# nikihowe/myriad

Hardware: AMD Instinct MI355X
Metric: converged trajopt solves/sec (batched), CARTPOLE collocation N=100 (higher is better)
Workload: dtype f64; 1 GPU; CARTPOLE HS collocation N=100, batch=4096 random x0 (weak), converged = status 0 and max|c|<=1e-8; global_batch=4096, parallelism=instances sharded over 1 GPU(s), one process per GPU

## Files before the change

### myriad_amd/csrc/hs_solver_fused.h

```cpp
#pragma once
#include <hip/hip_runtime.h>
#include "hs_solver_wave.h"

namespace myriad {

struct ParkArgs {
  int mode;
  int k1;
  const int* perm;
  const int* count;
  double* state;
  long stride;
};
constexpr int MYR_STATUS_PARKED_ = 5;

struct NodeBoard {
  unsigned long long cmd;
  unsigned int done;
  unsigned int xcc;
  unsigned int att;
  unsigned int pad_[27];
};
struct CoopArgs {
  NodeBoard* boards;
  double* pub;
  long pub_stride;
  int maxh;
  int* abort;
};
constexpr unsigned int MYR_COOP_RUNNING = 0x80000000u;
constexpr int MYR_COOP_EXIT = 15;
constexpr unsigned int MYR_COOP_GEN_MASK = 0x7fffu;
__device__ inline void coop_release() { asm volatile("s_waitcnt vmcnt(0) lgkmcnt(0)" ::: "memory"); }
__device__ inline void coop_acquire() { asm volatile("buffer_inv sc1\n\ts_waitcnt vmcnt(0)" ::: "memory"); }
#ifdef MYR_COOP_DEBUG
#define COOP_DBG(bit, ...) do { if ((MYR_COOP_DEBUG) & (bit)) printf(__VA_ARGS__); } while (0)
#else
#define COOP_DBG(bit, ...)
#endif
#ifdef MYR_COOP_TRACE
__device__ int* g_coop_trace;
#define COOP_TR(slot, val) do { if (g_coop_trace) __hip_atomic_store(g_coop_trace + blockIdx.x * 16 + (slot), (int)(val), __ATOMIC_RELAXED, __HIP_MEMORY_SCOPE_SYSTEM); } while (0)
#else
#define COOP_TR(slot, val)
#endif
__device__ inline unsigned int coop_xcc_id() { return __builtin_amdgcn_s_getreg((31 << 11) | 20) & 15u; }
constexpr unsigned MYR_COOP_SPIN_MAX = 1u << 23;

#ifdef MYR_PHASE_TIMING
__device__ long long node_tph_[8];
__device__ long long bw_tph_[4];
#define MYR_BW_PH(i) { if (blockIdx.x == 0 && c.tid == 0) { const long long t1_ = clock64(); bw_tph_[i] += t1_ - bw_t0_; bw_t0_ = t1_; } }
#else
#define MYR_BW_PH(i)
#endif

template <class Sys, int W = 1, int SCHEME = 0>
struct HsFused {
  static constexpr int NT = 64 * W;
  static constexpr bool TRAP = SCHEME == 1;
  using W0 = HsWave<Sys, 0>;
  using S = HsSolver<Sys>;
  using D = HsSol<Sys>;
  static constexpr int NS = D::NS, NU = D::NU, NW = D::NW, NY = TRAP ? NS + 2 * NU : D::NY, NQ = TRAP ? NU : D::NQ, NC = D::NC, NY1 = NY + 1;
  static constexpr int QE = NQ - NU;
#ifndef MYR_FWD_SEQ_NW
#define MYR_FWD_SEQ_NW 7
#endif
#ifndef MYR_TL_FLOOR
#define MYR_TL_FLOOR 1e-10
#endif
  static constexpr bool TL = W > 1 && NU == 1 && NS <= 4;
  static constexpr int MLAM = TRAP ? 1 : 2;
  static constexpr bool MLP = NodeTraits<Sys>::mlp;
  static_assert(!(MLP && TRAP), "network dynamics are built for the Hermite-Simpson transcription");
  static constexpr int PT_F = 0, PT_A = PT_F + NS, PT_B = PT_A + NS * NS, PT_D2 = PT_B + NS * NU, PT_N = PT_D2 + NW * (NW + 1) / 2;
  static constexpr int HSYM = NW * (NW + 1) / 2;
  static constexpr int HR_H = 0, HR_G0 = HSYM, HR_G1 = HR_G0 + NW, HR_N = HR_G1 + NW;
  static constexpr int SG_GE = 0, SG_GM = NS * NY1, SG_N = (TRAP ? 1 : 2) * NS * NY1;
  static constexpr int KST = NQ * NW + NQ * NC, KSTR = KST;
  static constexpr int ZR = 32;
  static constexpr int PF = MYR_RICCATI_PF;
  static constexpr int PADH = PF * 2 * HR_N, PADS = PF * SG_N;
  __host__ __device__ static constexpr int symidx(int r, int c) { return r <= c ? r * NW - r * (r - 1) / 2 + (c - r) : c * NW - c * (c - 1) / 2 + (r - c); }
  __host__ __device__ static constexpr int npoints(int N) { return TRAP ? N + 1 : 2 * N + 1; }
  __host__ __device__ static inline double wq(int K, int j, double h) {
    if (TRAP) return (j == 0 || j == K - 1) ? 0.5 * h : h;
    return S::wsimp(K, j, h);
  }
  __host__ __device__ static inline double tq(int j, double h) { return TRAP ? h * j : 0.5 * h * j; }

  __host__ __device__ static long off_hr(int) { return ZR + PADH; }
  __host__ __device__ static long off_st(int N) { return off_hr(N) + (long)npoints(N) * HR_N + PADS; }
  __host__ __device__ static long off_kg(int N) { return off_st(N) + (long)N * SG_N; }
  __host__ __device__ static long off_lam(int N) { return off_kg(N) + (long)N * KST; }
  __host__ __device__ static long off_kg2(int N) { return off_lam(N) + (long)MLAM * N * NS; }
  __host__ __device__ static long off_pt(int N) { return off_kg2(N) + (W > 1 ? (long)N * KST : 0); }
  __host__ __device__ static long off_hb(int N) { return off_pt(N) + (MLP ? (long)PT_N * npoints(N) : 0); }
  __host__ __device__ static long off_mb(int N) { return off_hb(N) + (MLP ? (long)NodeMfma64::ntiles(npoints(N)) * NodeMfma64::HB_TILE : 0); }
  __host__ __device__ static long off_zlu(int N) { return off_mb(N) + (MLP ? (long)NodeMfma64::ntiles(npoints(N)) * NodeMfma64::MB_TILE : 0); }
  static constexpr bool FSEQ = (MYR_FWD_SEQ_NW > 0) && NW >= MYR_FWD_SEQ_NW && !MLP;
  static constexpr int FWS = NW * NW + NW;
  __host__ __device__ static long off_fw(int N) { return off_zlu(N) + (ZLU_GLOBAL ? 2L * npoints(N) * NW : 0); }
  __host__ __device__ static long scratch_doubles(int N) { return off_fw(N) + (FSEQ ? (long)N * FWS : 0); }
  static constexpr int NREC = NS + NS + NS * NS + NS * NU + NS;
  static constexpr int EXCH = NW * NW + NW * NC + NS * NC + NU * NC;
  static constexpr int NTOT = NW * NW + NW, NRED = 12;
  static constexpr int XCH = 2 * W * NREC + 2 * W * NTOT + 2 * W * 2 * NS + W * NRED + 8;
  static constexpr int NCH = W;
  static constexpr int NXB = TL ? NCH : (W > 1 ? 2 : 1);
  static constexpr int TL_TH1 = NCH * NC, TL_JN1 = (NCH - 1) * 4 * NW * NW;
  static constexpr int TL_TH = TL ? TL_TH1 + (NCH + 1) + 2 : 0, TL_JN = TL ? TL_JN1 : 0;
  __host__ __device__ static constexpr int lds_solver_doubles_z(int N, bool zlu_global) { return (zlu_global ? 2 : 4) * npoints(N) * NW + MLAM * N * NS + 6 * NW + XCH + NXB * EXCH + TL_TH + TL_JN + 8; }
  static constexpr bool ZLU_GLOBAL = (MLP && W == 2) ||
      (!MLP && (MYR_FWD_SEQ_NW > 0) && NW >= MYR_FWD_SEQ_NW && (long)lds_solver_doubles_z(100, false) * 8 > 40960L * W);
  __host__ __device__ static int lds_solver_doubles(int N) { return lds_solver_doubles_z(N, ZLU_GLOBAL); }
  __host__ __device__ static int lds_doubles(int N) { return lds_solver_doubles(N) + (MLP ? npoints(N) * NS + NodeTraits<Sys>::lds_doubles : 0); }
  __host__ __device__ static size_t lds_bytes(int N) { return (size_t)lds_doubles(N) * 8; }
  static constexpr int NSCAL = 48;
  __host__ __device__ static long park_doubles(int N) { return NSCAL + lds_solver_doubles(N) + (ZLU_GLOBAL ? 2L * npoints(N) * NW : 0); }

  struct Ctx {
    int N, K, n, lane, wave, tid;
    double h, h6, h8;
    double *z, *zL, *zU, *dz;
    double *hr, *st, *kg, *zr;
    double *fw;
    double *kgA, *kgB, *xA, *xB;
    double *sTh, *sJn;
    double *pt, *sF, *wl;
    double *hb, *mb;
    int nh, hidx;
    unsigned int gen;
    NodeBoard* board; int* coop_abort;
    double *pubx, *publam, *pubf;
    bool h_valid;
    const double *lb, *ub;
    bool uni;
    SysParams<Sys> pp;
    bool term_pinned[NS];
    double *sLam, *sB, *sStash, *sTot, *sTr, *sRed, *sMisc, *sP, *sPc, *sTnu, *sKu;
#ifdef MYR_PHASE_TIMING
    long long tph[16], t0;
#endif
#ifdef MYR_TRACE
    int traj;
#endif
  };
  __device__ static inline long zi(const Ctx& c, int j, int comp) { return S::zi(c.K, j, comp); }
  __device__ static inline void use_set(Ctx& c, double* kg, double* x) {
    c.kg = kg; c.sP = x; c.sPc = x + NW * NW; c.sTnu = c.sPc + NW * NC; c.sKu = c.sTnu + NS * NC;
  }
  __device__ static inline void wsync() {
    __syncthreads();
  }
  template <int NV>
  __device__ static inline void wg_combine(Ctx& c, double* v, const int (&op)[NV]) {
    static_assert(NV <= NRED, "partial-sum slots");
    if constexpr (W > 1) {
#pragma unroll
      for (int i = 0; i < NV; ++i) c.sRed[c.wave * NRED + i] = v[i];
      __syncthreads();
#pragma unroll
      for (int i = 0; i < NV; ++i) {
        double r = c.sRed[i];
#pragma unroll
// ... 723 lines not shown
      for (int r = 0; r < NW; ++r) {
        const bool zr = last && r < NS && c.term_pinned[r < NS ? r : 0];
#pragma unroll
        for (int q = r; q < NW; ++q) {
          const bool zq = last && q < NS && c.term_pinned[q < NS ? q : 0];
          hr[HR_H + symidx(r, q)] = (zr || zq) ? 0.0 : (Wh[r * NW + q] + ((r == q) ? sig[r] : 0.0));
        }
        hr[HR_G0 + r] = zr ? 0.0 : (TL ? fma(mu_fold, g1v[r], wj * P.gw[r]) : wj * P.gw[r]);
        hr[HR_G1 + r] = zr ? 0.0 : g1v[r];
      }
      }
    }
    double v[1] = {wv_max(st_)};
    const int op[1] = {1};
    wg_combine<1>(c, v, op);
    stat = v[0];
  }

  __device__ static int riccati_first_point(Ctx& c, const HsSolveOpts& o, double delta, int nreg) {
    using namespace detail;
    const int lane = c.lane;
    const double* hr = c.hr;
    double Puu[NU * NU], ku[NU * NC], pun[NU * NS];
#pragma unroll
    for (int a = 0; a < NU; ++a) {
#pragma unroll
      for (int b = 0; b < NU; ++b) Puu[a * NU + b] = c.sP[(NS + a) * NW + NS + b] + hr[HR_H + symidx(NS + a, NS + b)] + ((a == b) ? delta : 0.0);
#pragma unroll
      for (int cc = 0; cc < NC; ++cc)
        ku[a * NC + cc] = c.sPc[(NS + a) * NC + cc] + (cc == 0 ? hr[HR_G0 + NS + a] : (cc == 1 ? hr[HR_G1 + NS + a] : 0.0));
#pragma unroll
      for (int i = 0; i < NS; ++i) pun[a * NS + i] = ku[a * NC + 2 + i];
    }
    nreg += chol_reg<NU>(Puu, o.reg_floor);
    chol_solve<NU, NC>(Puu, ku);
    wave_sync<true>();
    if (lane == 0) {
#pragma unroll
      for (int i = 0; i < NS; ++i)
#pragma unroll
        for (int cc = 0; cc < NC; ++cc) {
          double s = 0.0;
#pragma unroll
          for (int a = 0; a < NU; ++a) s += pun[a * NS + i] * ku[a * NC + cc];
          c.sTnu[i * NC + cc] -= s;
        }
#pragma unroll
      for (int i = 0; i < NU * NC; ++i) c.sKu[i] = ku[i];
    }
    wave_sync<true>();
    return nreg;
  }

  template <bool CHUNK>
  __device__ static int riccati_tile(Ctx& c, const HsSolveOpts& o, double delta, bool abort_on_reg, int k_lo_, int k_hi_, bool last_, double* xo) {
    using namespace detail;
    const int k_lo = CHUNK ? __builtin_amdgcn_readfirstlane(k_lo_) : 0, k_hi = __builtin_amdgcn_readfirstlane(CHUNK ? k_hi_ : c.N);
    const bool last = CHUNK ? last_ : true;
    static_assert(!CHUNK || (NC == NS + 2 && NU == 1), "slot 7 takes the control's multiplier");
    const int lane = c.lane;
    const int g = lane >> 4, j = lane & 15;
    const int scol = tile_scol<NS>(j), ycol = tile_ycol<NS, true>(j, scol), rcc = tile_rcc<NC>(j);
    const bool rowx = g < NS;
    const double* he = c.hr + (long)(2 * (k_hi - 1) + 2) * HR_N;
    const double* hm = he - HR_N;
    const double* st = c.st + (long)(k_hi - 1) * SG_N;
    auto hsel = [&](const double* rec, int row, bool on) -> const double* {
      if (!on) return c.zr;
      if (scol >= 0) return rec + HR_H + (scol <= row ? scol * NW - scol * (scol - 1) / 2 + (row - scol) : row * NW - row * (row - 1) / 2 + (scol - row));
      if (rcc == 0) return rec + HR_G0 + row;
      if constexpr (!CHUNK) { if (rcc == 1) return rec + HR_G1 + row; }
      return c.zr;
    };
    auto gsel = [&](int off) -> const double* {
      if (!rowx) return c.zr;
      if (ycol >= 0) return st + off + g * NY1 + ycol;
      if (rcc == 0) return st + off + g * NY1 + NY;
      return c.zr;
    };
    const double* ptr[6] = {hsel(he, g, rowx), hsel(he, NS, g < 2), gsel(SG_GE), hsel(hm, g, rowx), hsel(hm, NS, g < 2), gsel(SG_GM)};
    long stp[6];
#pragma unroll
    for (int q = 0; q < 6; ++q) stp[q] = (ptr[q] == c.zr) ? 0 : ((q == 2 || q == 5) ? (long)SG_N : 2L * HR_N);
    const bool pinr = rowx && (!last || c.term_pinned[rowx ? g : 0]);
    const double rho0 = last ? o.rho_term - delta : o.rho_term;
    double X0 = (pinr && scol == g) ? rho0 : ((pinr && rcc == 2 + g) ? 1.0 : 0.0);
    double X1 = (!last && g < 2) ? (scol == NS ? rho0 : (rcc == 1 ? 1.0 : 0.0)) : 0.0;
    const double dv0 = (rowx && scol == g) ? delta : 0.0, dv1 = (g < 2 && scol == NS) ? delta : 0.0;
    const TileMask<CHUNK, true> m(g, j, rcc);
    const int k_off = (g == 0 && scol >= 0 && j != 5) ? scol : ((g == 0 && rcc >= 0) ? NQ * NW + rcc : -1);
    const int k_str = k_off < 0 ? 1 : ((scol >= 0) ? NW : NC);
    double* k_ptr = k_off >= 0 ? c.kg + (long)(k_hi - 1) * KSTR + k_off : c.zr + ZR - 2;
    const long k_step = k_off >= 0 ? KSTR : 0;
    double reg_floor = o.reg_floor;
    asm volatile("" : "+v"(reg_floor));
    int nreg = 0;
    const bool abort_u = uniform_if<(W > 1)>(abort_on_reg);
    double in[PF][6];
#pragma unroll
    for (int u = 0; u < PF; ++u) {
#pragma unroll
      for (int q = 0; q < 6; ++q) { in[u][q] = *ptr[q]; ptr[q] -= stp[q]; }
      __builtin_amdgcn_sched_barrier(0);
    }
    mfma_d4 D1c = {0.0, 0.0, 0.0, 0.0}, Rmc = {0.0, 0.0, 0.0, 0.0};
    mfma_d4 Qm;
    double QmU;
    auto mid_part = [&](double n0, double n1, double Gm, const mfma_d4& Cup) -> mfma_d4 {
      const mfma_d4 Rm = tile_prod1<8>(n0 + dv0, n1 + dv1, Gm, m.f_a1, m.f_keep, m.f_shm, Cup);
      Qm = tile_mfma(Gm, Rm[0], mfma_d4{0.0, 0.0, 0.0, 0.0});
      QmU = Rm[1];
      return Rm;
    };
    mid_part(in[0][3], in[0][4], in[0][5], mfma_d4{0.0, 0.0, 0.0, 0.0});
    mfma_d4 D3 = {X0, X1, 0.0, 0.0};
    auto stage = [&](const int u) {
      X0 = D3[0] + (in[u][0] + dv0); X1 = fma(D3[1], m.f_x1, in[u][1] + dv1);
      const double G = in[u][2];
      const double nn0 = in[(u + 1) % PF][3], nn1 = in[(u + 1) % PF][4], nGm = in[(u + 1) % PF][5];
      const mfma_d4 D1 = tile_prod1<4>(X0, X1, G, m.f_a1, m.f_keep, m.f_she, D1c);
      D1c = D1;
      mfma_d4 C2 = tile_c2_hs(D3, D1, Qm, m.f_t1, m.f_t23);
      C2[3] += QmU;
      const mfma_d4 D2 = tile_mfma(G, D1[0], C2);
      Rmc = mid_part(nn0, nn1, nGm, Rmc);
      const TileGain2 gn = tile_gain2<(W > 1)>(D2, reg_floor, nreg, TileNoStop());
      k_ptr[0] = gn.kk0; k_ptr[k_str] = gn.kk1;
      k_ptr -= k_step;
      D3 = tile_update2(D2, gn.kk0, gn.kk1, m.f_a3m, m.f_a3e, g);
#pragma unroll
      for (int q = 0; q < 6; ++q) { in[u][q] = *ptr[q]; ptr[q] -= stp[q]; }
    };
    auto group = [&]() {
#pragma unroll
      for (int u = 0; u < PF; ++u) stage(u);
    };
    int kb = k_hi - 1;
    if (kb - k_lo >= PF - 1) {
      group();
      for (kb -= PF; kb - k_lo >= PF - 1; kb -= PF) {
        if (uniform_if<true>(nreg > 0 && abort_u)) return nreg;
        group();
      }
    }
#pragma unroll
    for (int u = 0; u < PF - 1; ++u) {
      if (kb - u < k_lo) break;
      stage(u);
    }
    if (uniform_if<true>(nreg > 0 && abort_u)) return nreg;
    if constexpr (!CHUNK) {
      tile_store_first<false, NS, NC>(D3, g, j, scol, rcc, rowx, c.sP, c.sPc, c.sTnu, [] { wave_sync<true>(); });
      return riccati_first_point(c, o, delta, nreg);
    } else {
      double* xP = xo; double* xPc = xo + NW * NW; double* xT = xPc + NW * NC;
      tile_store_first<true, NS, NC>(D3, g, j, scol, rcc, rowx, xP, xPc, xT, [] { wave_sync<true>(); });
      return nreg;
    }
  }

  static constexpr bool GEN = !(NU == 1 && NS <= 4);
  static constexpr bool G_BIG = NW > 8 || NQ > 8;
  static constexpr int G_QT = G_BIG ? 1 : 0;
  static constexpr int G_QS = G_BIG ? 16 : 8;
  static constexpr int G_NB = (NW + 3) / 4, G_NQB = (NQ + 3) / 4, G_NYT = G_QT + 1;
  static constexpr int G_FREE_LO = G_QS - NW, G_FREE_HI = 16 * (G_QT + 1) - G_QS - NQ;
  static constexpr int G_REST = NC - G_FREE_LO - G_FREE_HI;
  static constexpr int G_CT = G_QT + 1 + (G_REST > 0 ? 1 : 0);
  static constexpr bool GEN_OK = NW <= 14 && NQ <= 16 && (G_BIG ? G_FREE_LO : G_FREE_LO + G_FREE_HI) >= 2 && G_FREE_HI >= 0 && G_REST <= 16;
  static constexpr bool SUPPORTED = !GEN || GEN_OK;
  __host__ __device__ static constexpr int g_rhs_slot(int cc) {
    return cc < G_FREE_LO ? NW + cc : (cc - G_FREE_LO < G_FREE_HI ? G_QS + NQ + (cc - G_FREE_LO) : 16 * (G_QT + 1) + (cc - G_FREE_LO - G_FREE_HI));
  }
  __host__ __device__ static constexpr int g_slot_cc(int slot) {
    int cc = -1;
    if (slot < NW) cc = -1;
    else if (slot < G_QS) cc = slot - NW;
    else if (slot < G_QS + NQ) cc = -1;
    else if (slot < 16 * (G_QT + 1)) cc = G_FREE_LO + (slot - G_QS - NQ);
    else cc = G_FREE_LO + G_FREE_HI + (slot - 16 * (G_QT + 1));
    return cc < NC ? cc : -1;
  }
  __host__ __device__ static constexpr bool g_map_ok() {
    for (int cc = 0; cc < NC; ++cc)
      if (g_slot_cc(g_rhs_slot(cc)) != cc || g_rhs_slot(cc) >= 16 * G_CT) return false;
    return g_rhs_slot(0) < 16 && g_rhs_slot(1) < 16;
  }
  __device__ static int riccati_mfma_gen(Ctx& c, const HsSolveOpts& o, double delta, bool abort_on_reg) {
    using namespace detail;
    static_assert(GEN_OK && g_map_ok(), "slot map: w in front of the q, '1' and mu in the first column tile");
    constexpr int NB = G_NB, NQB = G_NQB, CT = G_CT, QT = G_QT, NYT = G_NYT;
    constexpr int QL = G_QS & 15;
    constexpr int QR = QL / 4;
    constexpr int PFG = G_BIG ? 2 : PF;
    constexpr int NL1 = NB * (1 + NYT);
    constexpr int NL = (TRAP ? 1 : 2) * NL1;
    constexpr int L_HE = 0, L_GE = NB, L_HM = NL1, L_GM = NL1 + NB;
    constexpr long H_STEP = TRAP ? (long)HR_N : 2L * HR_N;
    const int lane = c.lane, N = c.N;
    const int g = lane >> 4, j = lane & 15;
    int wc[CT], qc[CT], rc[CT], yc[NYT];
#pragma unroll
    for (int C = 0; C < CT; ++C) {
      const int slot = 16 * C + j;
      wc[C] = slot < NW ? slot : -1;
      qc[C] = (slot >= G_QS && slot < G_QS + NQ) ? slot - G_QS : -1;
      rc[C] = g_slot_cc(slot);
    }
#pragma unroll
    for (int C = 0; C < NYT; ++C) yc[C] = wc[C] >= 0 ? wc[C] : (qc[C] >= 0 ? NW + qc[C] : -1);
// ... 193 lines not shown
            }
        }
#pragma unroll
        for (int C = 0; C < CT; ++C)
#pragma unroll
          for (int b = 0; b < NQB; ++b) {
            double v = 0.0;
#pragma unroll
            for (int e = 0; e < 4; ++e)
              if (4 * b + e < NQ) v = (g == e) ? kk[C][4 * b + e] : v;
            kp[C][b][0] = v;
            kp[C][b] -= kstep[C][b];
          }
      }
    }
#pragma unroll
    for (int C = 0; C < CT; ++C) {
#pragma unroll
      for (int r = 0; r < NB; ++r) {
        const int row = 4 * r + g;
        if (row < NW && wc[C] >= 0) c.sP[row * NW + wc[C]] = Q[0][C][r];
        if (row < NW && rc[C] >= 0) c.sPc[row * NC + rc[C]] = Q[0][C][r];
      }
#pragma unroll
      for (int R = 0; R < CT; ++R)
#pragma unroll
        for (int r = 0; r < 4; ++r) {
          const int cc = g_slot_cc(16 * R + 4 * r + g);
          if (cc >= 2 && rc[C] >= 0) c.sTnu[(cc - 2) * NC + rc[C]] = Q[R][C][r];
        }
    }
    wave_sync<true>();
    {
      constexpr int s1 = g_rhs_slot(0);
      static_assert(s1 < 16, "row '1' in the first tile");
#pragma unroll
      for (int C = 0; C < CT; ++C)
        if (g == (s1 & 3) && rc[C] >= 2) c.sTnu[(rc[C] - 2) * NC + 0] += Q[0][C][s1 >> 2];
    }
    wave_sync<true>();
    return riccati_first_point(c, o, delta, nreg);
  }
  struct SwArgs { nd_glb *hr, *st, *zr, *kg; nd_lds* xs; int N, lane, pinned, abort; double reg_floor, rho_term, delta; };
  __device__ __attribute__((noinline)) static int sweep_call(SwArgs a) {
    Ctx c;
    c.N = a.N; c.lane = a.lane; c.hr = (double*)a.hr; c.st = (double*)a.st; c.zr = (double*)a.zr;
    use_set(c, (double*)a.kg, (double*)a.xs);
#pragma unroll
    for (int q = 0; q < NS; ++q) c.term_pinned[q] = ((a.pinned >> q) & 1) != 0;
    HsSolveOpts o;
    o.reg_floor = a.reg_floor; o.rho_term = a.rho_term;
    if constexpr (GEN) return riccati_mfma_gen(c, o, a.delta, a.abort != 0);
    else if constexpr (TRAP) return riccati_tile_trap<false>(c, o, a.delta, a.abort != 0, 0, 0, true, nullptr);
    else return riccati_tile<false>(c, o, a.delta, a.abort != 0, 0, 0, true, nullptr);
  }
  __device__ static inline int sweep(Ctx& c, const HsSolveOpts& o, double delta, bool abort_on_reg) {
#if !defined(MYR_SWEEP_CALL_W) || MYR_SWEEP_CALL_W
    constexpr bool CALL = true;
#else
    constexpr bool CALL = W == 1;
#endif
    if constexpr (!CALL) {
      if constexpr (GEN) return riccati_mfma_gen(c, o, delta, abort_on_reg);
      else if constexpr (TRAP) return riccati_tile_trap<false>(c, o, delta, abort_on_reg, 0, 0, true, nullptr);
      else return riccati_tile<false>(c, o, delta, abort_on_reg, 0, 0, true, nullptr);
    } else {
      SwArgs a;
      a.hr = (nd_glb*)c.hr; a.st = (nd_glb*)c.st; a.zr = (nd_glb*)c.zr; a.kg = (nd_glb*)c.kg; a.xs = (nd_lds*)c.sP;
      a.N = c.N; a.lane = c.lane; a.abort = abort_on_reg ? 1 : 0;
      a.pinned = 0;
#pragma unroll
      for (int q = 0; q < NS; ++q) a.pinned |= c.term_pinned[q] ? (1 << q) : 0;
      a.reg_floor = o.reg_floor; a.rho_term = o.rho_term; a.delta = delta;
      return sweep_call(a);
    }
  }

  template <bool CHUNK>
  __device__ static int riccati_tile_trap(Ctx& c, const HsSolveOpts& o, double delta, bool abort_on_reg, int k_lo_, int k_hi_, bool last_, double* xo) {
    using namespace detail;
    static_assert(!TRAP || NQ == 1, "one control");
    const int k_lo = CHUNK ? __builtin_amdgcn_readfirstlane(k_lo_) : 0, k_hi = __builtin_amdgcn_readfirstlane(CHUNK ? k_hi_ : c.N);
    const bool last = CHUNK ? last_ : true;
    const int lane = c.lane;
    const int g = lane >> 4, j = lane & 15;
    const int scol = tile_scol<NS>(j);
    const int ycol = scol >= 0 ? scol : ((j == 8 || j == 9) ? NW : -1);
    const int rcc = tile_rcc<NC>(j);
    const bool rowx = g < NS;
    const double* he = c.hr + (long)k_hi * HR_N;
    const double* st = c.st + (long)(k_hi - 1) * SG_N;
    auto hsel = [&](int row, bool on) -> const double* {
      if (!on) return c.zr;
      if (scol >= 0) return he + HR_H + (scol <= row ? scol * NW - scol * (scol - 1) / 2 + (row - scol) : row * NW - row * (row - 1) / 2 + (scol - row));
      if (rcc == 0) return he + HR_G0 + row;
      if constexpr (!CHUNK) { if (rcc == 1) return he + HR_G1 + row; }
      return c.zr;
    };
    const double* ptr[3] = {hsel(g, rowx), hsel(NS, g < 2),
                            !rowx ? c.zr : (ycol >= 0 ? st + SG_GE + g * NY1 + ycol : (rcc == 0 ? st + SG_GE + g * NY1 + NY : c.zr))};
    long stp[3];
#pragma unroll
    for (int q = 0; q < 3; ++q) stp[q] = (ptr[q] == c.zr) ? 0 : (q == 2 ? (long)SG_N : (long)HR_N);
    const bool pinr = rowx && (!last || c.term_pinned[rowx ? g : 0]);
    const double rho0 = last ? o.rho_term - delta : o.rho_term;
    const double X0i = (pinr && scol == g) ? rho0 : ((pinr && rcc == 2 + g) ? 1.0 : 0.0);
// ... 693 lines not shown
    wsync();
#pragma unroll
    for (int q = 0; q < NS; ++q) c.term_pinned[q] = !(c.sB[2 * NW + q] < c.sB[3 * NW + q]);
    res.status = 1; res.iters = o.max_iter;
    for (int it = it0; it <= o.max_iter; ++it) {
      if (park_mode == 1 && it == park_k1) {
        const int nl = lds_solver_doubles(c.N);
        for (int i = c.tid; i < nl; i += NT) __builtin_nontemporal_store(c.z[i], &sv[NSCAL + i]);
        if constexpr (ZLU_GLOBAL) {
          for (int i = c.tid; i < 2 * c.n; i += NT) __builtin_nontemporal_store(c.zL[i], &sv[NSCAL + nl + i]);
        }
        if (c.tid == 0) {
          s.save(sv, hist, pending);
          sv[PK_UNI] = c.uni ? 1.0 : 0.0;
          sv[PK_RES] = res.cost; sv[PK_RES + 1] = res.feas; sv[PK_RES + 2] = res.stat; sv[PK_RES + 3] = res.compl_;
        }
        res.status = MYR_STATUS_PARKED_; res.iters = it;
        return;
      }
      if constexpr (MLP) { if (c.board) coop_refresh(c); }
      BOut p1;
      { NuT nu_; for (int q = 0; q < NS; ++q) nu_.v[q] = s.nuT[q]; p1 = backward_pass(c, pending, nu_); }
      pending.on = false;
      c.h_valid = false;
      wsync();
      MYR_PH(0)
      double stat_raw;
      const double mu_hess = s.mu;
      stat_raw = hessian_pass(c, s.mu);
      wsync();
      MYR_PH(4)
      const double c1 = p1.c1, cinf = p1.cinf, sum_mult = p1.sum_mult;
      double delta = s.first_delta(o);
      int nreg = 0;
      {
        const IpKkt k = s.kkt(o, sum_mult + p1.sm, MLAM * c.N * NS + p1.nm, p1.f, stat_raw, p1.cmax, cinf);
        res.cost = p1.f; res.feas = cinf; res.stat = k.stat; res.compl_ = k.comp;
        if (__builtin_amdgcn_readfirstlane((int)!k.finite)) { res.status = 2; res.iters = it; return; }
        if (__builtin_amdgcn_readfirstlane((int)k.converged)) { res.status = 0; res.iters = it; return; }
        if (it == o.max_iter) break;
        s.barrier_update(o, k, cinf, p1.cmin, p1.cmax);
      }
#if !defined(MYR_FUSED_SPEC) || MYR_FUSED_SPEC
      constexpr bool SPEC = W > 1;
#else
      constexpr bool SPEC = false;
#endif
      if constexpr (TL) {
        if (__builtin_amdgcn_readfirstlane((int)(s.mu != mu_hess))) {
          tl_fold(c, s.mu - mu_hess);
          wsync();
        }
        MYR_PH(3)
        double* cnt = c.sTh + TL_TH1;
        for (int tr_ = 0; tr_ < 12; ++tr_) {
          const bool abort_on_reg = s.rung_aborts(tr_, delta);
          int nr = 0;
          if (tl_edge(c.N, c.wave + 1) > tl_edge(c.N, c.wave)) nr = sweep_chunk(c, o, delta, abort_on_reg, c.wave);
          cnt[c.wave] = (double)nr;
          MYR_PH(13)
          wsync();
          MYR_PH(5)
          int ns = 0;
#pragma unroll
          for (int w = 0; w < W; ++w) ns += (int)cnt[w];
          ns = __builtin_amdgcn_readfirstlane(ns);
          if (ns == 0 || !abort_on_reg) {
            if (c.wave == 0) {
              JnArgs ja;
              ja.xb = (nd_lds*)c.xA; ja.jn = (nd_lds*)c.sJn; ja.N = c.N; ja.lane = c.lane; ja.rho = o.rho_term; ja.floor_c = MYR_TL_FLOOR;
              int nj = tl_join(ja);
              MYR_PH(9)
              nj = riccati_first_point(c, o, delta, nj);
              cnt[W] = (double)nj;
              MYR_PH(10)
            }
            wsync();
            ns += (int)cnt[W];
          }
          nreg = __builtin_amdgcn_readfirstlane(ns);
#ifdef MYR_TRACE
          if (c.tid == 0 && c.traj < MYR_TRACE) {
            printf("L b%d it%d rung %d delta=%.9g chunks", c.traj, it, tr_, delta);
            for (int w = 0; w < W; ++w) printf(" %d", (int)cnt[w]);
            printf(" join+first %d\n", (ns == nreg && ((int)cnt[0] + (W > 1 ? (int)cnt[1] : 0)) == 0) ? (int)cnt[W] : -1);
          }
#endif
          wsync();
          MYR_PH(6)
          if (nreg == 0 || !abort_on_reg) break;
          delta = s.next_delta(delta);
        }
      } else
      if constexpr (SPEC) {
        use_set(c, c.kgA, c.xA);
        for (int tr_ = 0; tr_ < 12; tr_ += 2) {
          const double delta_b = s.next_delta(delta);
          const bool abort_a = s.rung_aborts(tr_, delta), abort_b = s.rung_aborts(tr_ + 1, delta_b);
          {
            Ctx cw = c;
            if (c.wave == 1) use_set(cw, c.kgB, c.xB);
            if (c.wave < 2) {
              const int nr = sweep(cw, o, c.wave == 0 ? delta : delta_b, c.wave == 0 ? abort_a : abort_b);
              c.sMisc[1 + c.wave] = (double)nr;
            }
          }
          wsync();
          const int na = (int)c.sMisc[1], nb = (int)c.sMisc[2];
          wsync();
          MYR_PH(6)
          nreg = na;
          if (na == 0 || !abort_a) break;
          delta = delta_b; nreg = nb;
          if (nb == 0 || !abort_b) {
            for (int i = c.tid; i < c.N * KST; i += NT) c.kgA[i] = c.kgB[i];
            for (int i = c.tid; i < EXCH; i += NT) c.xA[i] = c.xB[i];
            wsync();
            break;
          }
          delta = s.next_delta(delta_b);
        }
      } else {
        for (int tr_ = 0; tr_ < 12; ++tr_) {
          const bool abort_on_reg = s.rung_aborts(tr_, delta);
          if constexpr (W > 1) {
            if (c.wave == 0) {
              nreg = sweep(c, o, delta, abort_on_reg);
              c.sMisc[1] = (double)nreg;
            }
            wsync();
            nreg = (int)c.sMisc[1];
          } else nreg = sweep(c, o, delta, abort_on_reg);
          wsync();
          MYR_PH(6)
          if (nreg == 0) break;
          if (!abort_on_reg) break;
          delta = s.next_delta(delta);
        }
      }
      s.close_ladder(delta);
#ifdef MYR_TRACE
      if (c.lane == 0 && c.traj < MYR_TRACE)
        printf("T b%d w%d it%d f=%.17g c1=%.17g cinf=%.17g stat=%.17g sm=%.17g lg=%.17g nreg=%d delta=%.9g mu=%.9g pen=%.9g\n", c.traj, c.wave, it,
               p1.f, p1.c1, p1.cinf, stat_raw, p1.sum_mult, p1.lg, nreg, delta, s.mu, s.pen);
#endif
      typename S::SweepOut so;
#pragma unroll
      for (int i = 0; i < NS * NC; ++i) so.Tnu[i] = c.sTnu[i];
#pragma unroll
      for (int i = 0; i < NS; ++i) so.term_pinned[i] = c.term_pinned[i];
      double nu[NS];
      S::solve_nu(so, TL ? 0.0 : s.mu, nu);
      double th[NC];
      th[0] = 1.0; th[1] = TL ? 0.0 : s.mu;
#pragma unroll
      for (int i = 0; i < NS; ++i) th[2 + i] = nu[i];
      if constexpr (TL) {
        if (c.wave == 0) tl_theta(c, th);
        wsync();
      }
      MYR_PH(7)
      typename S::FwdOut fo;
      { ThT th_; for (int q = 0; q < NC; ++q) th_.v[q] = th[q]; fo = forward_pass(c, o, s.mu, th_); }
      wsync();
      MYR_PH(8)
      if (!(finite_(fo.gphi) && finite_(fo.alpha_p))) { res.status = 2; res.iters = it; return; }
      const double Dphi = s.penalty_update(fo.gphi, c1);
      const double f0 = p1.f, bar0 = s.mu * p1.lg, c10 = c1;
      const double phi0 = f0 + bar0 + s.pen * c10;
      const double phiref = s.merit_reference(o, hist, phi0);
      double a = fo.alpha_p;
      bool ok = false;
      for (int ls = 0; ls < 40; ++ls) {
        const TrialOut tr1 = trial_pass(c, a, s.mu);
        if (tr1.ok && s.accepts(tr1.f + tr1.bar + s.pen * tr1.c1, phiref, a, Dphi, phi0)) { ok = true; break; }
        a *= 0.5;
      }
      if (s.stalled(ok)) { res.status = 3; res.iters = it; return; }
      c.h_valid = ok;
      MYR_PH(11)
#ifdef MYR_TRACE
      if (c.lane == 0 && c.traj < MYR_TRACE)
        printf("S b%d w%d it%d ap=%.17g ad=%.17g gphi=%.17g a=%.17g ok=%d nu0=%.17g\n", c.traj, c.wave, it, fo.alpha_p, fo.alpha_d, fo.gphi, a, (int)ok, nu[0]);
#endif
      pending.on = true; pending.ap = a; pending.ad = s.dual_step(o, a, fo.alpha_p, fo.alpha_d); pending.mu = s.mu;
#pragma unroll
      for (int i = 0; i < NS; ++i) s.follow_nu(i, a, nu[i]);
      s.after_step(o, a, fo.alpha_p);
      wsync();
    }
    res.status = 1; res.iters = o.max_iter;
  }
};

template <class Sys, int NWAVES = 1, int SCHEME = 0>
__global__ __launch_bounds__(64 * NWAVES, 1)
void hs_solve_fused_kernel(int B, int* ticket, HsSolveOpts o, VarScale vs, double* __restrict__ z, const double* __restrict__ lb,
                           const double* __restrict__ ub, double* lam, double* scratch, long scratch_stride,
                           const double* __restrict__ params, int params_stride, double* cost, int32_t* status,
                           int32_t* iters, double* kkt, unsigned long long poison, ParkArgs pk, CoopArgs co) {
  using W = HsFused<Sys, NWAVES, SCHEME>;
  extern __shared__ __attribute__((aligned(16))) char smem_fused[];
  typename W::Ctx c;
  c.N = o.N; c.K = W::npoints(o.N); c.n = c.K * W::NW; c.lane = threadIdx.x & 63; c.tid = threadIdx.x;
  c.wave = __builtin_amdgcn_readfirstlane(threadIdx.x >> 6);
  c.h = o.h; c.h6 = o.h / 6.0; c.h8 = o.h / 8.0;
  const bool coop = W::MLP && co.maxh > 0;
  const bool fixed = coop && B <= (int)gridDim.x;
  const int nboards = fixed ? B : (int)gridDim.x;
  const bool can_own = !fixed || (int)blockIdx.x < B;
  c.nh = 0; c.hidx = 0;
  c.board = (coop && can_own) ? co.boards + blockIdx.x : nullptr; c.coop_abort = co.abort;
  c.pubx = (coop && can_own) ? co.pub + (long)blockIdx.x * co.pub_stride : nullptr;
  c.publam = c.pubx ? c.pubx + c.n : nullptr; c.pubf = c.pubx ? c.publam + W::MLAM * c.N * W::NS : nullptr;
  double* s = scratch + (long)(can_own ? blockIdx.x : 0u) * scratch_stride;
  c.zr = s; c.hr = s + W::off_hr(c.N); c.st = s + W::off_st(c.N); c.kg = s + W::off_kg(c.N);
  c.kgA = c.kg; c.kgB = s + W::off_kg2(c.N); c.pt = s + W::off_pt(c.N);
  c.hb = s + W::off_hb(c.N); c.mb = s + W::off_mb(c.N); c.h_valid = false;
  c.fw = s + W::off_fw(c.N);
  double* const lam_own = s + W::off_lam(c.N);
  double* l = reinterpret_cast<double*>(smem_fused);
  c.z = l; l += c.n;
  if constexpr (W::ZLU_GLOBAL) { c.zL = s + W::off_zlu(c.N); c.zU = c.zL + c.n; }
  else { c.zL = l; l += c.n; c.zU = l; l += c.n; }
  c.dz = l; l += c.n;
  c.sLam = l; l += W::MLAM * c.N * W::NS;
  c.sB = l; l += 6 * W::NW;
  c.sStash = l; l += 2 * NWAVES * W::NREC;
  c.sTot = l; l += 2 * NWAVES * W::NTOT;
  c.sTr = l; l += 2 * NWAVES * 2 * W::NS;
  c.sRed = l; l += NWAVES * W::NRED;
  c.sMisc = l; l += 8;
  c.xA = l; c.xB = l + W::EXCH;
  c.sTh = l + W::NXB * W::EXCH; c.sJn = c.sTh + W::TL_TH;
  W::use_set(c, c.kgA, c.xA);
  c.sF = reinterpret_cast<double*>(smem_fused) + W::lds_solver_doubles(c.N);
  c.wl = c.sF + c.K * W::NS;
  if constexpr (W::MLP) {
    if (params_stride == 0) {
      SysParams<Sys> pw;
      pw.load(params, 0, 0);
      NodeMfma64::load_weights(pw.get(), c.wl, c.tid, W::NT);
      __syncthreads();
    }
  }
  if constexpr (W::MLP) {
    if (coop) {
      if (c.tid == 0) {
        W::coop_seq(c) = 0; W::coop_target(c) = 0;
        if (c.board) __hip_atomic_store(&c.board->xcc, 1u + coop_xcc_id(), __ATOMIC_RELAXED, __HIP_MEMORY_SCOPE_AGENT);
      }
      __syncthreads();
    }
  }
  bool took = false;
  c.gen = 0;
  for (;;) {
    int t = 0;
    if (c.tid == 0) t = fixed ? ((can_own && !took) ? (int)blockIdx.x : B) : atomicAdd(ticket, 1);
    took = true;
    if constexpr (NWAVES > 1) {
      if (c.tid == 0) reinterpret_cast<int*>(c.sMisc)[0] = t;
      __syncthreads();
      t = reinterpret_cast<int*>(c.sMisc)[0];
    }
    long b = __builtin_amdgcn_readfirstlane(t);
    if (pk.mode == 2) {
      if (b >= pk.count[0]) break;
      b = pk.perm[b];
    } else if (b >= B) break;
    double* zg = z + b * (long)c.n;
    c.lb = lb + b * (long)c.n; c.ub = ub + b * (long)c.n;
    double* lamg = lam ? lam + b * (long)(W::MLAM * c.N * W::NS) : lam_own;
    if (poison) {
      __syncthreads();
      const unsigned int keep_seq = W::coop_seq(c), keep_target = W::coop_target(c);
      __syncthreads();
      double* l0 = reinterpret_cast<double*>(smem_fused);
      const int nl = W::lds_solver_doubles(c.N) + (W::MLP ? c.K * W::NS : 0);
      const unsigned long long salt = (unsigned long long)b * 1315423911ULL + blockIdx.x;
      for (int i = c.tid; i < nl; i += W::NT) l0[i] = poison_value(poison, (unsigned long long)i, salt);
      for (long i = c.tid; i < scratch_stride; i += W::NT) s[i] = poison_value(poison, (unsigned long long)i + (1ULL << 32), salt);
      __syncthreads();
      if (c.tid == 0) { W::coop_seq(c) = keep_seq; W::coop_target(c) = keep_target; }
      __syncthreads();
    }
#ifdef MYR_TRACE
    c.traj = (int)b;
#endif
    c.pp.load(params, b, params_stride);
    c.pp.set_scale(vs.s);
    if constexpr (W::MLP) {
      if (params_stride != 0) {
        NodeMfma64::load_weights(c.pp.get(), c.wl, c.tid, W::NT);
        __syncthreads();
      }
    }
    HsSolveResult r;
#ifdef MYR_PHASE_TIMING
    for (int i = 0; i < 16; ++i) c.tph[i] = 0;
    c.t0 = clock64();
#endif
    if constexpr (W::MLP) {
      c.nh = 0;
      c.gen = (c.gen + 1u) & MYR_COOP_GEN_MASK;
      if (coop && c.tid == 0) {
        __hip_atomic_store(&c.board->att, MYR_COOP_RUNNING | (c.gen << 16), __ATOMIC_RELAXED, __HIP_MEMORY_SCOPE_AGENT);
      }
    }
    if constexpr (NWAVES == 1 || W::MLP) W::solve(c, o, zg, r, pk.mode, pk.k1, pk.state + b * pk.stride);
    else W::solve(c, o, zg, r);
    if (r.status != MYR_STATUS_PARKED_) {
      for (int i = c.tid; i < c.n; i += W::NT) zg[i] = c.z[i];
      for (int i = c.tid; i < W::MLAM * c.N * W::NS; i += W::NT) lamg[i] = c.sLam[i];
    }
#ifdef MYR_PHASE_TIMING
    if (c.lane == 0 && b < 4) {
      printf("traj %ld wave %d it %d: backward %lld hess %lld fold %lld chunk %lld wait %lld join %lld first %lld ricc %lld nu %lld forward %lld ls %lld\n",
             b, c.wave, r.iters, c.tph[0], c.tph[4], c.tph[3], c.tph[13], c.tph[5], c.tph[9], c.tph[10], c.tph[6], c.tph[7], c.tph[8], c.tph[11]);
    }
    if (!W::MLP && c.tid == 0 && blockIdx.x == 0) {
      printf("  workgroup 0, traj %ld it %d: backward pass in parts (cycles): linearisation %lld stage maps %lld scan + multipliers %lld\n", b, r.iters, bw_tph_[0], bw_tph_[1], bw_tph_[2]);
      bw_tph_[0] = bw_tph_[1] = bw_tph_[2] = 0;
    }
    if (W::MLP && c.tid == 0 && blockIdx.x == 0) {
      printf("  workgroup 0, traj %ld it %d: network passes of wavefront 0 (cycles): MODE0 %lld MODE3 %lld MODE4 %lld\n", b, r.iters, node_tph_[0], node_tph_[3], node_tph_[4]);
      node_tph_[0] = node_tph_[3] = node_tph_[4] = 0;
      for (int m = 0; m < 5; m += (m == 0 ? 3 : 1)) {
        printf("    MODE %d segments: inputs %lld | layer 1 + sigmoids %lld | layer 2 %lld | sigmoids 2 %lld | activations stored / loaded %lld | last layer %lld | tangents / contraction %lld\n", m,
               node_seg_[m][0], node_seg_[m][1], node_seg_[m][2], node_seg_[m][3], node_seg_[m][4], node_seg_[m][5], node_seg_[m][6]);
        for (int q = 0; q < 8; ++q) node_seg_[m][q] = 0;
      }
    }
#endif
    if (c.tid == 0) {
      if (cost) cost[b] = r.cost;
      if (status) status[b] = r.status;
      if (iters) iters[b] = r.iters;
      if (kkt) { kkt[3 * b] = r.feas; kkt[3 * b + 1] = r.stat; kkt[3 * b + 2] = r.compl_; }
    }
    W::wsync();
    if constexpr (W::MLP) {
      if (coop) {
        if (c.tid == 0) {
          (void)__hip_atomic_exchange(&c.board->att, 0u, __ATOMIC_RELAXED, __HIP_MEMORY_SCOPE_AGENT);
          coop_release();
          const unsigned int seq = ++W::coop_seq(c);
          __hip_atomic_store(&c.board->cmd, ((unsigned long long)seq << 32) | ((unsigned long long)c.gen << 16) | (unsigned long long)MYR_COOP_EXIT, __ATOMIC_RELAXED, __HIP_MEMORY_SCOPE_AGENT);
          coop_release();
          (void)__hip_atomic_fetch_add(co.abort + 1, 1, __ATOMIC_RELAXED, __HIP_MEMORY_SCOPE_AGENT);
        }
        c.nh = 0;
        __syncthreads();
      }
    }
  }
  if constexpr (W::MLP) {
    if (coop) {
      typename W::HelpArgs ha;
      ha.N = c.N; ha.K = c.K; ha.n = c.n; ha.lane = c.lane; ha.wave = c.wave; ha.tid = c.tid; ha.h6 = c.h6; ha.h8 = c.h8;
      ha.z = c.z; ha.sLam = c.sLam; ha.sF = c.sF; ha.wl = c.wl; ha.sMisc = c.sMisc;
      ha.co = co; ha.scratch = scratch; ha.scratch_stride = scratch_stride; ha.B = B; ha.nboards = nboards;
      W::coop_help(ha);
    }
  }
}

}
```

Measured before the change: 347,700 solves/s.

## Run single-wave Riccati sweep as two interleaved chunks joined afterward

For single-wave Hermite-Simpson solves with small state (cartpole), the backward Riccati recursion is split into two independent chunks. Both chunks are swept within one wavefront, with their dependent MFMA chains interleaved so that each hides the other's latency, and the results are joined with the existing chunk-join plus first-point step. LDS layout is reshuffled, with exchange buffers aliased onto dz and unused multi-wave buffers dropped. The join adds extra work and numerical-conditioning risk, and it raises register pressure from the doubled prefetch state.

```diff
diff --git a/myriad_amd/csrc/hs_solver_fused.h b/myriad_amd/csrc/hs_solver_fused.h
--- a/myriad_amd/csrc/hs_solver_fused.h
+++ b/myriad_amd/csrc/hs_solver_fused.h
@@ -51,9 +51,18 @@
 __device__ long long node_tph_[8];
 __device__ long long bw_tph_[4];
 #define MYR_BW_PH(i) { if (blockIdx.x == 0 && c.tid == 0) { const long long t1_ = clock64(); bw_tph_[i] += t1_ - bw_t0_; bw_t0_ = t1_; } }
+#define MYR_SW_T0 const long long sw_t0_ = clock64();
+#define MYR_SW_T1(done) { if (done) { c.tph[14] += clock64() - sw_t0_; c.tph[15] += 1; } }
 #else
 #define MYR_BW_PH(i)
+#define MYR_SW_T0
+#define MYR_SW_T1(done)
 #endif
+
+#ifndef MYR_PAIRED_SWEEP
+#define MYR_PAIRED_SWEEP 1
+#endif
+template <class Sys> struct PairedSweep { static constexpr bool value = MYR_PAIRED_SWEEP != 0; };
 
 template <class Sys, int W = 1, int SCHEME = 0>
 struct HsFused {
@@ -70,9 +79,11 @@
 #ifndef MYR_TL_FLOOR
 #define MYR_TL_FLOOR 1e-10
 #endif
-  static constexpr bool TL = W > 1 && NU == 1 && NS <= 4;
   static constexpr int MLAM = TRAP ? 1 : 2;
   static constexpr bool MLP = NodeTraits<Sys>::mlp;
+  static constexpr bool PAIR = W == 1 && !TRAP && !MLP && NU == 1 && NS <= 4 && PairedSweep<Sys>::value;
+  static constexpr bool TL = (W > 1 || PAIR) && NU == 1 && NS <= 4;
+  static constexpr bool UNI = W > 1 || PAIR;
   static_assert(!(MLP && TRAP), "network dynamics are built for the Hermite-Simpson transcription");
   static constexpr int PT_F = 0, PT_A = PT_F + NS, PT_B = PT_A + NS * NS, PT_D2 = PT_B + NS * NU, PT_N = PT_D2 + NW * (NW + 1) / 2;
   static constexpr int HSYM = NW * (NW + 1) / 2;
@@ -106,12 +117,16 @@
   static constexpr int NREC = NS + NS + NS * NS + NS * NU + NS;
   static constexpr int EXCH = NW * NW + NW * NC + NS * NC + NU * NC;
   static constexpr int NTOT = NW * NW + NW, NRED = 12;
-  static constexpr int XCH = 2 * W * NREC + 2 * W * NTOT + 2 * W * 2 * NS + W * NRED + 8;
-  static constexpr int NCH = W;
+  static constexpr int XCH = 2 * W * NREC + (W > 1 ? 2 * W * NTOT + 2 * W * 2 * NS : 0) + W * NRED + 8;
+  static constexpr int NCH = PAIR ? 2 : W;
   static constexpr int NXB = TL ? NCH : (W > 1 ? 2 : 1);
   static constexpr int TL_TH1 = NCH * NC, TL_JN1 = (NCH - 1) * 4 * NW * NW;
   static constexpr int TL_TH = TL ? TL_TH1 + (NCH + 1) + 2 : 0, TL_JN = TL ? TL_JN1 : 0;
-  __host__ __device__ static constexpr int lds_solver_doubles_z(int N, bool zlu_global) { return (zlu_global ? 2 : 4) * npoints(N) * NW + MLAM * N * NS + 6 * NW + XCH + NXB * EXCH + TL_TH + TL_JN + 8; }
+  static constexpr int NXR = PAIR ? 1 : NXB;
+  __host__ __device__ static constexpr int dz_doubles(int N) { return (PAIR && npoints(N) * NW < EXCH + TL_JN) ? EXCH + TL_JN : npoints(N) * NW; }
+  __host__ __device__ static constexpr int lds_solver_doubles_z(int N, bool zlu_global) {
+    return (zlu_global ? 1 : 3) * npoints(N) * NW + dz_doubles(N) + MLAM * N * NS + 6 * NW + XCH + NXR * EXCH + TL_TH + (PAIR ? 0 : TL_JN) + 8;
+  }
   static constexpr bool ZLU_GLOBAL = (MLP && W == 2) ||
       (!MLP && (MYR_FWD_SEQ_NW > 0) && NW >= MYR_FWD_SEQ_NW && (long)lds_solver_doubles_z(100, false) * 8 > 40960L * W);
   __host__ __device__ static int lds_solver_doubles(int N) { return lds_solver_doubles_z(N, ZLU_GLOBAL); }
@@ -941,19 +956,21 @@
     return nreg;
   }
 
-  template <bool CHUNK>
+  template <bool CHUNK, int NP = 1>
   __device__ static int riccati_tile(Ctx& c, const HsSolveOpts& o, double delta, bool abort_on_reg, int k_lo_, int k_hi_, bool last_, double* xo) {
     using namespace detail;
+    static_assert(NP == 1 || (NP == 2 && CHUNK), "a pair is two chunks");
     const int k_lo = CHUNK ? __builtin_amdgcn_readfirstlane(k_lo_) : 0, k_hi = __builtin_amdgcn_readfirstlane(CHUNK ? k_hi_ : c.N);
     const bool last = CHUNK ? last_ : true;
     static_assert(!CHUNK || (NC == NS + 2 && NU == 1), "slot 7 takes the control's multiplier");
+    int klo[NP], khi[NP];
+    bool lastp[NP];
+    if constexpr (NP == 1) { klo[0] = k_lo; khi[0] = k_hi; lastp[0] = last; }
+    else { klo[0] = 0; khi[0] = k_lo; lastp[0] = false; klo[1] = k_lo; khi[1] = k_hi; lastp[1] = true; }
     const int lane = c.lane;
     const int g = lane >> 4, j = lane & 15;
     const int scol = tile_scol<NS>(j), ycol = tile_ycol<NS, true>(j, scol), rcc = tile_rcc<NC>(j);
     const bool rowx = g < NS;
-    const double* he = c.hr + (long)(2 * (k_hi - 1) + 2) * HR_N;
-    const double* hm = he - HR_N;
-    const double* st = c.st + (long)(k_hi - 1) * SG_N;
     auto hsel = [&](const double* rec, int row, bool on) -> const double* {
       if (!on) return c.zr;
       if (scol >= 0) return rec + HR_H + (scol <= row ? scol * NW - scol * (scol - 1) / 2 + (row - scol) : row * NW - row * (row - 1) / 2 + (scol - row));
@@ -961,90 +978,138 @@
       if constexpr (!CHUNK) { if (rcc == 1) return rec + HR_G1 + row; }
       return c.zr;
     };
-    auto gsel = [&](int off) -> const double* {
+    auto gsel = [&](const double* st, int off) -> const double* {
       if (!rowx) return c.zr;
       if (ycol >= 0) return st + off + g * NY1 + ycol;
       if (rcc == 0) return st + off + g * NY1 + NY;
       return c.zr;
     };
-    const double* ptr[6] = {hsel(he, g, rowx), hsel(he, NS, g < 2), gsel(SG_GE), hsel(hm, g, rowx), hsel(hm, NS, g < 2), gsel(SG_GM)};
+    const double* ptr[NP][6];
+#pragma unroll
+    for (int p = 0; p < NP; ++p) {
+      const double* he = c.hr + (long)(2 * (khi[p] - 1) + 2) * HR_N;
+      const double* hm = he - HR_N;
+      const double* st = c.st + (long)(khi[p] - 1) * SG_N;
+      ptr[p][0] = hsel(he, g, rowx); ptr[p][1] = hsel(he, NS, g < 2); ptr[p][2] = gsel(st, SG_GE);
+      ptr[p][3] = hsel(hm, g, rowx); ptr[p][4] = hsel(hm, NS, g < 2); ptr[p][5] = gsel(st, SG_GM);
+    }
     long stp[6];
 #pragma unroll
-    for (int q = 0; q < 6; ++q) stp[q] = (ptr[q] == c.zr) ? 0 : ((q == 2 || q == 5) ? (long)SG_N : 2L * HR_N);
-    const bool pinr = rowx && (!last || c.term_pinned[rowx ? g : 0]);
-    const double rho0 = last ? o.rho_term - delta : o.rho_term;
-    double X0 = (pinr && scol == g) ? rho0 : ((pinr && rcc == 2 + g) ? 1.0 : 0.0);
-    double X1 = (!last && g < 2) ? (scol == NS ? rho0 : (rcc == 1 ? 1.0 : 0.0)) : 0.0;
+    for (int q = 0; q < 6; ++q) stp[q] = (ptr[0][q] == c.zr) ? 0 : ((q == 2 || q == 5) ? (long)SG_N : 2L * HR_N);
     const double dv0 = (rowx && scol == g) ? delta : 0.0, dv1 = (g < 2 && scol == NS) ? delta : 0.0;
     const TileMask<CHUNK, true> m(g, j, rcc);
     const int k_off = (g == 0 && scol >= 0 && j != 5) ? scol : ((g == 0 && rcc >= 0) ? NQ * NW + rcc : -1);
     const int k_str = k_off < 0 ? 1 : ((scol >= 0) ? NW : NC);
-    double* k_ptr = k_off >= 0 ? c.kg + (long)(k_hi - 1) * KSTR + k_off : c.zr + ZR - 2;
+    double* k_ptr[NP];
+#pragma unroll
+    for (int p = 0; p < NP; ++p) k_ptr[p] = k_off >= 0 ? c.kg + (long)(khi[p] - 1) * KSTR + k_off : c.zr + ZR - 2;
     const long k_step = k_off >= 0 ? KSTR : 0;
     double reg_floor = o.reg_floor;
     asm volatile("" : "+v"(reg_floor));
-    int nreg = 0;
-    const bool abort_u = uniform_if<(W > 1)>(abort_on_reg);
-    double in[PF][6];
+    int nreg[NP];
+    const bool abort_u = uniform_if<UNI>(abort_on_reg);
+    mfma_d4 D3[NP];
+#pragma unroll
+    for (int p = 0; p < NP; ++p) {
+      nreg[p] = 0;
+      const bool pinr = rowx && (!lastp[p] || c.term_pinned[rowx ? g : 0]);
+      const double rho0 = lastp[p] ? o.rho_term - delta : o.rho_term;
+      const double X0 = (pinr && scol == g) ? rho0 : ((pinr && rcc == 2 + g) ? 1.0 : 0.0);
+      const double X1 = (!lastp[p] && g < 2) ? (scol == NS ? rho0 : (rcc == 1 ? 1.0 : 0.0)) : 0.0;
+      D3[p] = mfma_d4{X0, X1, 0.0, 0.0};
+    }
+    const bool odd = NP == 2 && (khi[NP - 1] - klo[NP - 1]) > (khi[0] - klo[0]);
+    double ex[6];
+    if constexpr (NP == 2) {
+      if (odd) {
+#pragma unroll
+        for (int q = 0; q < 6; ++q) { ex[q] = *ptr[1][q]; ptr[1][q] -= stp[q]; }
+      }
+    }
+    double in[NP][PF][6];
 #pragma unroll
     for (int u = 0; u < PF; ++u) {
 #pragma unroll
-      for (int q = 0; q < 6; ++q) { in[u][q] = *ptr[q]; ptr[q] -= stp[q]; }
+      for (int p = 0; p < NP; ++p)
+#pragma unroll
+        for (int q = 0; q < 6; ++q) { in[p][u][q] = *ptr[p][q]; ptr[p][q] -= stp[q]; }
       __builtin_amdgcn_sched_barrier(0);
     }
-    mfma_d4 D1c = {0.0, 0.0, 0.0, 0.0}, Rmc = {0.0, 0.0, 0.0, 0.0};
-    mfma_d4 Qm;
-    double QmU;
-    auto mid_part = [&](double n0, double n1, double Gm, const mfma_d4& Cup) -> mfma_d4 {
+    mfma_d4 D1c[NP], Rmc[NP], Qm[NP], D2[NP];
+    double QmU[NP];
+    auto mid_part = [&](const int p, double n0, double n1, double Gm, const mfma_d4& Cup) -> mfma_d4 {
       const mfma_d4 Rm = tile_prod1<8>(n0 + dv0, n1 + dv1, Gm, m.f_a1, m.f_keep, m.f_shm, Cup);
-      Qm = tile_mfma(Gm, Rm[0], mfma_d4{0.0, 0.0, 0.0, 0.0});
-      QmU = Rm[1];
+      Qm[p] = tile_mfma(Gm, Rm[0], mfma_d4{0.0, 0.0, 0.0, 0.0});
+      QmU[p] = Rm[1];
       return Rm;
     };
-    mid_part(in[0][3], in[0][4], in[0][5], mfma_d4{0.0, 0.0, 0.0, 0.0});
-    mfma_d4 D3 = {X0, X1, 0.0, 0.0};
+    auto front = [&](const int p, double c0, double c1, double G, double nn0, double nn1, double nGm) {
+      const double X0 = D3[p][0] + (c0 + dv0), X1 = fma(D3[p][1], m.f_x1, c1 + dv1);
+      const mfma_d4 D1 = tile_prod1<4>(X0, X1, G, m.f_a1, m.f_keep, m.f_she, D1c[p]);
+      D1c[p] = D1;
+      mfma_d4 C2 = tile_c2_hs(D3[p], D1, Qm[p], m.f_t1, m.f_t23);
+      C2[3] += QmU[p];
+      D2[p] = tile_mfma(G, D1[0], C2);
+      Rmc[p] = mid_part(p, nn0, nn1, nGm, Rmc[p]);
+    };
+    auto back = [&](const int p) {
+      const TileGain2 gn = tile_gain2<UNI>(D2[p], reg_floor, nreg[p], TileNoStop());
+      k_ptr[p][0] = gn.kk0; k_ptr[p][k_str] = gn.kk1;
+      k_ptr[p] -= k_step;
+      D3[p] = tile_update2(D2[p], gn.kk0, gn.kk1, m.f_a3m, m.f_a3e, g);
+    };
+#pragma unroll
+    for (int p = 0; p < NP; ++p) { D1c[p] = mfma_d4{0.0, 0.0, 0.0, 0.0}; Rmc[p] = mfma_d4{0.0, 0.0, 0.0, 0.0}; }
+    mid_part(0, in[0][0][3], in[0][0][4], in[0][0][5], mfma_d4{0.0, 0.0, 0.0, 0.0});
+    if constexpr (NP == 2) {
+      if (odd) {
+        mid_part(1, ex[3], ex[4], ex[5], mfma_d4{0.0, 0.0, 0.0, 0.0});
+        front(1, ex[0], ex[1], ex[2], in[1][0][3], in[1][0][4], in[1][0][5]);
+        back(1);
+      } else
+        mid_part(1, in[1][0][3], in[1][0][4], in[1][0][5], mfma_d4{0.0, 0.0, 0.0, 0.0});
+    }
     auto stage = [&](const int u) {
-      X0 = D3[0] + (in[u][0] + dv0); X1 = fma(D3[1], m.f_x1, in[u][1] + dv1);
-      const double G = in[u][2];
-      const double nn0 = in[(u + 1) % PF][3], nn1 = in[(u + 1) % PF][4], nGm = in[(u + 1) % PF][5];
-      const mfma_d4 D1 = tile_prod1<4>(X0, X1, G, m.f_a1, m.f_keep, m.f_she, D1c);
-      D1c = D1;
-      mfma_d4 C2 = tile_c2_hs(D3, D1, Qm, m.f_t1, m.f_t23);
-      C2[3] += QmU;
-      const mfma_d4 D2 = tile_mfma(G, D1[0], C2);
-      Rmc = mid_part(nn0, nn1, nGm, Rmc);
-      const TileGain2 gn = tile_gain2<(W > 1)>(D2, reg_floor, nreg, TileNoStop());
-      k_ptr[0] = gn.kk0; k_ptr[k_str] = gn.kk1;
-      k_ptr -= k_step;
-      D3 = tile_update2(D2, gn.kk0, gn.kk1, m.f_a3m, m.f_a3e, g);
-#pragma unroll
-      for (int q = 0; q < 6; ++q) { in[u][q] = *ptr[q]; ptr[q] -= stp[q]; }
+#pragma unroll
+      for (int p = 0; p < NP; ++p)
+        front(p, in[p][u][0], in[p][u][1], in[p][u][2], in[p][(u + 1) % PF][3], in[p][(u + 1) % PF][4], in[p][(u + 1) % PF][5]);
+#pragma unroll
+      for (int p = 0; p < NP; ++p) back(p);
+#pragma unroll
+      for (int p = 0; p < NP; ++p)
+#pragma unroll
+        for (int q = 0; q < 6; ++q) { in[p][u][q] = *ptr[p][q]; ptr[p][q] -= stp[q]; }
     };
+    auto failed = [&]() { int n = 0; for (int p = 0; p < NP; ++p) n += nreg[p]; return n; };
     auto group = [&]() {
 #pragma unroll
       for (int u = 0; u < PF; ++u) stage(u);
     };
-    int kb = k_hi - 1;
-    if (kb - k_lo >= PF - 1) {
+    const int s_lo = klo[0];
+    int kb = khi[0] - 1;
+    if (kb - s_lo >= PF - 1) {
       group();
-      for (kb -= PF; kb - k_lo >= PF - 1; kb -= PF) {
-        if (uniform_if<true>(nreg > 0 && abort_u)) return nreg;
+      for (kb -= PF; kb - s_lo >= PF - 1; kb -= PF) {
+        if (uniform_if<true>(failed() > 0 && abort_u)) return failed();
         group();
       }
     }
 #pragma unroll
     for (int u = 0; u < PF - 1; ++u) {
-      if (kb - u < k_lo) break;
+      if (kb - u < s_lo) break;
       stage(u);
     }
-    if (uniform_if<true>(nreg > 0 && abort_u)) return nreg;
+    if (uniform_if<true>(failed() > 0 && abort_u)) return failed();
     if constexpr (!CHUNK) {
-      tile_store_first<false, NS, NC>(D3, g, j, scol, rcc, rowx, c.sP, c.sPc, c.sTnu, [] { wave_sync<true>(); });
-      return riccati_first_point(c, o, delta, nreg);
+      tile_store_first<false, NS, NC>(D3[0], g, j, scol, rcc, rowx, c.sP, c.sPc, c.sTnu, [] { wave_sync<true>(); });
+      return riccati_first_point(c, o, delta, nreg[0]);
     } else {
-      double* xP = xo; double* xPc = xo + NW * NW; double* xT = xPc + NW * NC;
-      tile_store_first<true, NS, NC>(D3, g, j, scol, rcc, rowx, xP, xPc, xT, [] { wave_sync<true>(); });
-      return nreg;
+#pragma unroll
+      for (int p = 0; p < NP; ++p) {
+        double* xP = xo + p * EXCH; double* xPc = xP + NW * NW; double* xT = xPc + NW * NC;
+        tile_store_first<true, NS, NC>(D3[p], g, j, scol, rcc, rowx, xP, xPc, xT, [] { wave_sync<true>(); });
+      }
+      return failed();
     }
   }
 
@@ -1344,6 +1409,7 @@
     o.reg_floor = a.reg_floor; o.rho_term = a.rho_term;
     if constexpr (GEN) return riccati_mfma_gen(c, o, a.delta, a.abort != 0);
     else if constexpr (TRAP) return riccati_tile_trap<false>(c, o, a.delta, a.abort != 0, 0, 0, true, nullptr);
+    else if constexpr (PAIR) return riccati_tile<true, 2>(c, o, a.delta, a.abort != 0, tl_edge(a.N, 1), a.N, true, (double*)a.xs);
     else return riccati_tile<false>(c, o, a.delta, a.abort != 0, 0, 0, true, nullptr);
   }
   __device__ static inline int sweep(Ctx& c, const HsSolveOpts& o, double delta, bool abort_on_reg) {
@@ -2143,6 +2209,28 @@
           wsync();
         }
         MYR_PH(3)
+        if constexpr (PAIR) {
+          for (int tr_ = 0; tr_ < 12; ++tr_) {
+            const bool abort_on_reg = s.rung_aborts(tr_, delta);
+            MYR_SW_T0
+            int ns = sweep(c, o, delta, abort_on_reg);
+            MYR_SW_T1(ns == 0 || !abort_on_reg)
+            MYR_PH(13)
+            if (ns == 0 || !abort_on_reg) {
+              JnArgs ja;
+              ja.xb = (nd_lds*)c.xA; ja.jn = (nd_lds*)c.sJn; ja.N = c.N; ja.lane = c.lane; ja.rho = o.rho_term; ja.floor_c = MYR_TL_FLOOR;
+              int nj = tl_join(ja);
+              MYR_PH(9)
+              ns += riccati_first_point(c, o, delta, nj);
+              MYR_PH(10)
+            }
+            nreg = __builtin_amdgcn_readfirstlane(ns);
+            wsync();
+            MYR_PH(6)
+            if (nreg == 0 || !abort_on_reg) break;
+            delta = s.next_delta(delta);
+          }
+        } else {
         double* cnt = c.sTh + TL_TH1;
         for (int tr_ = 0; tr_ < 12; ++tr_) {
           const bool abort_on_reg = s.rung_aborts(tr_, delta);
@@ -2181,6 +2269,7 @@
           MYR_PH(6)
           if (nreg == 0 || !abort_on_reg) break;
           delta = s.next_delta(delta);
+        }
         }
       } else
       if constexpr (SPEC) {
@@ -2221,7 +2310,11 @@
             }
             wsync();
             nreg = (int)c.sMisc[1];
-          } else nreg = sweep(c, o, delta, abort_on_reg);
+          } else {
+            MYR_SW_T0
+            nreg = sweep(c, o, delta, abort_on_reg);
+            MYR_SW_T1(nreg == 0 || !abort_on_reg)
+          }
           wsync();
           MYR_PH(6)
           if (nreg == 0) break;
@@ -2247,6 +2340,7 @@
 #pragma unroll
       for (int i = 0; i < NS; ++i) th[2 + i] = nu[i];
       if constexpr (TL) {
+        MYR_PH(12)
         if (c.wave == 0) tl_theta(c, th);
         wsync();
       }
@@ -2314,16 +2408,19 @@
   c.z = l; l += c.n;
   if constexpr (W::ZLU_GLOBAL) { c.zL = s + W::off_zlu(c.N); c.zU = c.zL + c.n; }
   else { c.zL = l; l += c.n; c.zU = l; l += c.n; }
-  c.dz = l; l += c.n;
+  if constexpr (W::PAIR) { c.xA = l; l += W::EXCH; }
+  c.dz = l; l += W::dz_doubles(c.N);
   c.sLam = l; l += W::MLAM * c.N * W::NS;
   c.sB = l; l += 6 * W::NW;
   c.sStash = l; l += 2 * NWAVES * W::NREC;
-  c.sTot = l; l += 2 * NWAVES * W::NTOT;
-  c.sTr = l; l += 2 * NWAVES * 2 * W::NS;
+  if constexpr (NWAVES > 1) {
+    c.sTot = l; l += 2 * NWAVES * W::NTOT;
+    c.sTr = l; l += 2 * NWAVES * 2 * W::NS;
+  } else { c.sTot = nullptr; c.sTr = nullptr; }
   c.sRed = l; l += NWAVES * W::NRED;
   c.sMisc = l; l += 8;
-  c.xA = l; c.xB = l + W::EXCH;
-  c.sTh = l + W::NXB * W::EXCH; c.sJn = c.sTh + W::TL_TH;
+  if constexpr (W::PAIR) { c.xB = c.dz; c.sJn = c.dz + W::EXCH; c.sTh = l; }
+  else { c.xA = l; c.xB = l + W::EXCH; c.sTh = l + W::NXB * W::EXCH; c.sJn = c.sTh + W::TL_TH; }
   W::use_set(c, c.kgA, c.xA);
   c.sF = reinterpret_cast<double*>(smem_fused) + W::lds_solver_doubles(c.N);
   c.wl = c.sF + c.K * W::NS;
@@ -2407,8 +2504,10 @@
     }
 #ifdef MYR_PHASE_TIMING
     if (c.lane == 0 && b < 4) {
-      printf("traj %ld wave %d it %d: backward %lld hess %lld fold %lld chunk %lld wait %lld join %lld first %lld ricc %lld nu %lld forward %lld ls %lld\n",
-             b, c.wave, r.iters, c.tph[0], c.tph[4], c.tph[3], c.tph[13], c.tph[5], c.tph[9], c.tph[10], c.tph[6], c.tph[7], c.tph[8], c.tph[11]);
+      printf("traj %ld wave %d it %d: backward %lld hess %lld fold %lld chunk %lld wait %lld join %lld first %lld ricc %lld nu %lld theta %lld forward %lld ls %lld\n",
+             b, c.wave, r.iters, c.tph[0], c.tph[4], c.tph[3], c.tph[13], c.tph[5], c.tph[9], c.tph[10], c.tph[6], W::TL ? c.tph[12] : c.tph[7], W::TL ? c.tph[7] : 0LL,
+             c.tph[8], c.tph[11]);
+      if (NWAVES == 1) printf("traj %ld: %lld sweeps ran to their end in %lld cycles (first point included unless the form joins chunks)\n", b, c.tph[15], c.tph[14]);
     }
     if (!W::MLP && c.tid == 0 && blockIdx.x == 0) {
       printf("  workgroup 0, traj %ld it %d: backward pass in parts (cycles): linearisation %lld stage maps %lld scan + multipliers %lld\n", b, r.iters, bw_tph_[0], bw_tph_[1], bw_tph_[2]);
```

After: 279,500 solves/s. 19.6% lower.
